# philip-bl/dctn

Hardware: AMD Instinct MI355X
Metric: EPS-contraction windows/sec (fwd+bwd) (higher is better)
Workload: dtype bf16; 1 GPU; cfg2 EPS[(3,4)]+linear bf16 B1024/GPU; parallelism=dp1

## Files before the change

### dctn_amd/_lib.py

```python
from __future__ import annotations

import ctypes
import os
import subprocess
from typing import Optional, Sequence

import torch

_HERE = os.path.dirname(os.path.abspath(__file__))
LIB_PATH = os.path.join(_HERE, "libdctn_amd.so")
CSRC = os.path.join(_HERE, "csrc")

F32, F64, BF16 = 0, 1, 2
PREC_EXACT, PREC_BF16, PREC_SPLIT, PREC_MASK = 0, 1, 2, 0xFF
OPT_F32_PREFER_HALVES, OPT_SMALL_CHUNKS, OPT_MAIN_KERNEL_ONLY, OPT_GENERIC_KERNELS = 1 << 8, 1 << 9, 1 << 10, 1 << 11
OPT_HEAD_FEATURES_BLOCKED4 = 1 << 12
ERR_BAD_SHAPE, ERR_BAD_DTYPE, ERR_UNSUPPORTED, ERR_WORKSPACE, ERR_LAUNCH, ERR_NULL = -1, -2, -3, -4, -5, -6
SAVED, PARTIAL = 1, 2
(EPS_FAMILY_GENERIC, EPS_FAMILY_Q2REG, EPS_FAMILY_BIGCORE_F32, EPS_FAMILY_HALVES, EPS_FAMILY_Q2REG_F32,
 EPS_FAMILY_BIGCORE_BF16X3) = range(6)
SBS_MATRIX_CORE_SWEEP = 1 << 8
SBS_WIDE_SWEEP = 1 << 9

_DTYPE_CODE = {torch.float32: F32, torch.float64: F64, torch.bfloat16: BF16}

c_int, c_i64, c_void, c_size = ctypes.c_int, ctypes.c_int64, ctypes.c_void_p, ctypes.c_size_t
_I64x5 = ctypes.POINTER(c_i64)
_IntP = ctypes.POINTER(c_int)
_PtrP = ctypes.POINTER(c_void)

SIGNATURES = {
    "dctn_version": (c_int, []),
    "dctn_strerror": (ctypes.c_char_p, [c_int]),
    "dctn_last_kernel": (ctypes.c_char_p, []),
    "dctn_device_limits": (c_int, [_IntP, _IntP]),
    "dctn_eps_family": (c_int, [c_int] * 9),
    "dctn_eps_fwd_workspace_bytes": (c_size, [c_int] * 7 + [c_int] * 2),
    "dctn_eps_fwd": (c_int, [c_void, _I64x5, c_void, c_void, c_void, c_size] + [c_int] * 7 + [c_int, c_int, c_void]),
    "dctn_eps_saved_bytes": (c_size, [c_int] * 7 + [c_int] * 2),
# ... 216 lines not shown
```

### dctn_amd/csrc/capi.hip

```cpp
#include "common.h"

#include <stdio.h>
#include <stdlib.h>

#include <algorithm>
#include <atomic>

static std::atomic<const char*> g_last_kernel{"none"};
void dctn_set_last_kernel(const char* name) { g_last_kernel.store(name, std::memory_order_relaxed); }

const DctnDev& dctn_dev() {
  static const DctnDev d = [] {
    DctnDev r{256, 160 * 1024};
    int dev = 0, v = 0;
    if (hipGetDevice(&dev) == hipSuccess) {
      if (hipDeviceGetAttribute(&v, hipDeviceAttributeMultiprocessorCount, dev) == hipSuccess && v > 0) r.cus = v;
      if (hipDeviceGetAttribute(&v, hipDeviceAttributeMaxSharedMemoryPerMultiprocessor, dev) == hipSuccess && v >= 64 * 1024) r.lds = v;
    }
    int cus = 0, lds = 0;
    const char* lim = getenv("DCTN_DEVICE_LIMITS");
    if (lim && sscanf(lim, "%d,%d", &cus, &lds) == 2) {
      if (cus > 0 && cus < r.cus) r.cus = cus;
      if (lds > 0 && lds < r.lds) r.lds = lds;
    }
// ... 121 lines not shown
  r.fwd_saving = r.fwd[0] == DCTN_EPS_FAMILY_Q2REG_F32 && r.saved_layout == EPS_SAVED_Z && r.saved_bytes > 0;
  r.dcore_reg = q2reg ? DCTN_EPS_FAMILY_Q2REG : q2f32 ? DCTN_EPS_FAMILY_Q2REG_F32 : EPS_NO_FAMILY;
  r.dcore_reg_saved = q2reg ? DCTN_EPS_FAMILY_Q2REG : EPS_NO_FAMILY;
  if (r.saved_layout == EPS_SAVED_HALVES)
    eps_list(r.bwd, DCTN_EPS_FAMILY_HALVES, DCTN_EPS_FAMILY_BIGCORE_F32, DCTN_EPS_FAMILY_GENERIC);
  else
    eps_list(r.bwd, DCTN_EPS_FAMILY_BIGCORE_F32, DCTN_EPS_FAMILY_GENERIC);
  return r;
}

static int eps_fwd_family(int family, const void* x, const void* core, void* out, void* ws, size_t ws_bytes, const EpsP& p,
                          int dtype, const EpsRoute& r, hipStream_t st, void* keep) {
  switch (family) {
    case DCTN_EPS_FAMILY_BIGCORE_BF16X3: return eps_fwd_bf16x3(x, core, out, ws, ws_bytes, p, dtype, DCTN_PREC_SPLIT, st, keep);
    case DCTN_EPS_FAMILY_Q2REG: return eps_fwd_mfma(x, core, out, p, dtype, r.precision, st);
    case DCTN_EPS_FAMILY_Q2REG_F32: return eps_fwd_q2f32(x, core, out, p, dtype, r.precision, st);
    case DCTN_EPS_FAMILY_BIGCORE_F32: return eps_fwd_bigcore(x, core, out, ws, ws_bytes, p, dtype, r.precision, st, keep);
    case DCTN_EPS_FAMILY_HALVES: return eps_fwd_halves(x, core, out, ws, ws_bytes, p, dtype, st, keep);
  }
  return eps_fwd_generic(x, core, out, p, dtype, st);
}

static int eps_head_params(EpsP& p, const int64_t x_strides[5], int C, int B, int H, int W, int Q, int K, int O, int Cout,
                           int dtype, int policy) {
  if (!dtype_ok(dtype)) return DCTN_ERR_BAD_DTYPE;
  if (Cout < 1) return DCTN_ERR_BAD_SHAPE;
  const int blk = policy & DCTN_OPT_HEAD_FEATURES_BLOCKED4;
  const int rc = eps_fill_params(p, x_strides, C, B, H, W, Q, K, O, policy & ~blk);
  p.opts |= blk;
  return rc;
}

static bool eps_head_next(const EpsP& p, int rc) {
  return rc == DCTN_ERR_UNSUPPORTED && !(p.opts & DCTN_OPT_HEAD_FEATURES_BLOCKED4);
}

extern "C" {

int dctn_version(void) { return 500; }

const char* dctn_last_kernel(void) { return g_last_kernel.load(std::memory_order_relaxed); }

int dctn_device_limits(int* cus, int* lds_bytes) {
  if (!cus || !lds_bytes) return DCTN_ERR_NULL;
  *cus = dctn_dev().cus;
  *lds_bytes = dctn_dev().lds;
  return DCTN_OK;
}

const char* dctn_strerror(int code) {
// ... 112 lines not shown
  if (need_dx) b = std::max(b, eps_bwd_dfactor_bigcore_workspace(p, dtype, r.precision));
  if (need_dcore) b = std::max(b, eps_bwd_dcore_bigcore_workspace(p, dtype, r.precision));
  return a + b + 256;
}

int dctn_eps_head_fwd(const void* x, const int64_t x_strides[5], const void* core, const void* head_weight,
                      const void* head_bias, void* features, void* logits, int C, int B, int H, int W, int Q, int K, int O,
                      int Cout, int dtype, int policy, void* stream) {
  if (!x || !core || !head_weight || !head_bias || !features || !logits || !x_strides) return DCTN_ERR_NULL;
  EpsP p;
  int rc = eps_head_params(p, x_strides, C, B, H, W, Q, K, O, Cout, dtype, policy);
  if (rc != DCTN_OK) return rc;
  const int precision = policy & DCTN_PREC_MASK;
  hipStream_t st = (hipStream_t)stream;
  rc = eps_head_fwd_mfma(x, core, head_weight, head_bias, features, logits, p, Cout, dtype, precision, st);
  if (!eps_head_next(p, rc)) return rc;
  return eps_head_fwd_q2f32(x, core, head_weight, head_bias, features, logits, p, Cout, dtype, precision, st);
}

size_t dctn_eps_head_bwd_workspace_bytes(int C, int B, int H, int W, int Q, int K, int O, int Cout, int dtype,
                                         int policy) {
  EpsP p;
  const int precision = policy & DCTN_PREC_MASK;
  if (!eps_query_params(p, C, B, H, W, Q, K, O, policy & ~DCTN_OPT_HEAD_FEATURES_BLOCKED4)) return 0;
  const size_t a = eps_head_bwd_mfma_workspace(p, Cout, dtype, precision), b = eps_head_bwd_q2f32_workspace(p, Cout, dtype, precision);
  return (a > b ? a : b) + 256;
}

int dctn_eps_head_bwd(const void* x, const int64_t x_strides[5], const void* features, const void* dLogits,
                      const void* head_weight, void* dCore, void* dWeight, void* dBias, void* workspace,
                      size_t workspace_bytes, int C, int B, int H, int W, int Q, int K, int O, int Cout,
                      int dtype, int policy, void* stream) {
  if (!x || !features || !dLogits || !head_weight || !dCore || !x_strides) return DCTN_ERR_NULL;
  EpsP p;
  int rc = eps_head_params(p, x_strides, C, B, H, W, Q, K, O, Cout, dtype, policy);
  if (rc != DCTN_OK) return rc;
  const int precision = policy & DCTN_PREC_MASK;
  hipStream_t st = (hipStream_t)stream;
  rc = eps_head_bwd_mfma(x, features, dLogits, head_weight, dCore, dWeight, dBias, workspace, workspace_bytes, p, Cout, dtype,
                         precision, st);
  if (!eps_head_next(p, rc)) return rc;
  return eps_head_bwd_q2f32(x, features, dLogits, head_weight, dCore, dWeight, dBias, workspace, workspace_bytes, p, Cout, dtype,
                            precision, st);
}

static int eps_bwd_impl(const void* x, const int64_t x_strides[5], const void* core, const void* dY, const void* saved,
                        size_t saved_bytes, void* dX, void* dCore, void* workspace, size_t workspace_bytes, int C, int B,
                        int H, int W, int Q, int K, int O, int dtype, int policy, void* stream) {
  if (!x || !core || !dY || !x_strides) return DCTN_ERR_NULL;
  if (!dtype_ok(dtype)) return DCTN_ERR_BAD_DTYPE;
  if (!dX && !dCore) return DCTN_OK;
  EpsP p;
  int rc = eps_fill_params(p, x_strides, C, B, H, W, Q, K, O, policy);
  if (rc != DCTN_OK) return rc;
  hipStream_t st = (hipStream_t)stream;
  const EpsRoute r = eps_route(p, dtype, policy);
  unsigned char* ws = (unsigned char*)workspace;
  size_t ws_bytes = workspace_bytes;
// ... 64 lines not shown
```

### dctn_amd/csrc/eps_generic.hip

```cpp
#include "common.h"

namespace {

template <typename S>
__device__ __forceinline__ typename AccOf<S>::type ldv(const S* p) {
  return (typename AccOf<S>::type)(*p);
}

struct WinCoord {
  long long b;
  int ho, wo;
};

__device__ __forceinline__ WinCoord win_coord(const EpsP& p, long long w) {
  WinCoord c;
  const int hw = p.Ho * p.Wo;
  c.b = w / hw;
  const int rem = (int)(w - c.b * hw);
  c.ho = rem / p.Wo;
  c.wo = rem - c.ho * p.Wo;
  return c;
}

template <typename S, typename A>
// ... 263 lines not shown
      }
    }
    if (rvalid) {
#pragma unroll
      for (int j = 0; j < OT; ++j)
        if (o0 + j < p.O) atomicAdd(&dCoreAcc[row * p.O + o0 + j], acc[j]);
    }
  }
}

}

template <typename S, typename A>
__global__ void convert_k(const A* __restrict__ src, S* __restrict__ dst, long long n) {
  for (long long i = (long long)blockIdx.x * blockDim.x + threadIdx.x; i < n;
       i += (long long)gridDim.x * blockDim.x)
    dst[i] = (S)src[i];
}
template __global__ void convert_k<bf16_t, float>(const float*, bf16_t*, long long);

int eps_fill_params(EpsP& p, const int64_t xs[5], int C, int B, int H, int W, int Q, int K, int O, int policy) {
  p.opts = policy & ~DCTN_PREC_MASK;
  if ((p.opts & ~DCTN_OPT_ALL) || (policy & DCTN_PREC_MASK) > DCTN_PREC_SPLIT || policy < 0) return DCTN_ERR_UNSUPPORTED;
  if (p.opts & DCTN_OPT_HEAD_FEATURES_BLOCKED4) return DCTN_ERR_UNSUPPORTED;
  if (C < 1 || B < 1 || Q < 1 || K < 1 || O < 1 || H < K || W < K) return DCTN_ERR_BAD_SHAPE;
  p.C = C; p.B = B; p.H = H; p.W = W; p.Q = Q; p.K = K; p.O = O;
  p.N = K * K * C;
  p.Ho = H - K + 1;
  p.Wo = W - K + 1;
  p.Wn = (long long)B * p.Ho * p.Wo;
  long long R = 1;
  for (int n = 0; n < p.N; ++n) {
    R *= Q;
    if (R > (1LL << 40)) return DCTN_ERR_UNSUPPORTED;
  }
  p.R = R;
  for (int i = 0; i < 5; ++i) p.s[i] = xs[i];
  int m = 0;
  long long lo = 1;
  while (m < p.N && lo * Q <= 32) { lo *= Q; ++m; }
  p.m = m; p.LO = (int)lo; p.NH = p.N - m;
  p.HI = ipow_ll(Q, p.NH);
  p.bits = Q <= 16 ? 4 : 8;
  return DCTN_OK;
}

static size_t fwd_lds(const EpsP& p, size_t asz) {
// ... 153 lines not shown
```

### dctn_amd/csrc/eps_mfma.hip

```cpp
#include "common.h"

#include <cstdlib>
#include <type_traits>

typedef __attribute__((ext_vector_type(8))) __bf16 bf16x8;
typedef __attribute__((ext_vector_type(16))) float f32x16;
typedef __attribute__((ext_vector_type(8))) float f32x8;
typedef __attribute__((ext_vector_type(2))) int int2v;
typedef __attribute__((ext_vector_type(4))) int int4v;
typedef __attribute__((ext_vector_type(2))) float f32x2;

namespace {

constexpr int ilog2(int v) { return v <= 1 ? 0 : 1 + ilog2(v >> 1); }

template <typename S> __device__ __forceinline__ float to_f32(S v) { return (float)v; }

__device__ __forceinline__ float half_sum(float v) {
  const int iv = __float_as_int(v);
  const int2v r = __builtin_amdgcn_permlane32_swap(iv, iv, false, false);
  return __int_as_float(r[0]) + __int_as_float(r[1]);
}

__device__ __forceinline__ void swap_halves(float& a, float& b) {
// ... 51 lines not shown
__device__ __forceinline__ unsigned fdiv(unsigned n, const FastDiv& d) {
  const unsigned t = __umulhi(d.M, n);
  return (t + ((n - t) >> d.s1)) >> d.s2;
}

#define MFMA_MAXN 16
struct MfmaP {
  int C, B, K, O, Ho, Wo;
  int P;
  int npg;
  int spc, nchunks;
  unsigned foffb[MFMA_MAXN];
  unsigned rowoffb[MFMA_MAXN];
  unsigned s1b, s2b, s3b, s4b;
  unsigned x_bytes;
  unsigned o_bytes, o_s1b;
  FastDiv div_wo;
  int rowvec_ok;
  int vec_ok;
  int Cout;
  unsigned hw_rowb, hw_bytes;
  int ncb;
  int opts;
#ifdef DCTN_STAMPS
  unsigned long long* stamps;
#endif
};

#ifdef DCTN_STAMPS
#define DCTN_STAMP(P, SLOT)                                                                      \
  do {                                                                                           \
    __builtin_amdgcn_sched_barrier(0);                                                           \
    unsigned long long t_;                                                                       \
    asm volatile("s_memrealtime %0\n\ts_waitcnt lgkmcnt(0)" : "=s"(t_)::"memory");               \
    if ((P).stamps && threadIdx.x == 0) (P).stamps[(long long)blockIdx.x * 8 + (SLOT)] = t_;     \
    __builtin_amdgcn_sched_barrier(0);                                                           \
  } while (0)
static unsigned long long* g_stamps = nullptr;
void dctn_stamps_set(unsigned long long* p) { g_stamps = p; }
__device__ unsigned long long* g_dev_stamps = nullptr;
void dctn_reduce_stamps_set(unsigned long long* p) { (void)hipMemcpyToSymbol(HIP_SYMBOL(g_dev_stamps), &p, sizeof(p)); }
#define DCTN_STAMP_T(P, SLOT, TID)                                                              \
  do {                                                                                           \
    __builtin_amdgcn_sched_barrier(0);                                                           \
    unsigned long long t_;                                                                       \
    asm volatile("s_memrealtime %0\n\ts_waitcnt lgkmcnt(0)" : "=s"(t_)::"memory");               \
// ... 178 lines not shown
        __builtin_amdgcn_raw_buffer_store_b128(u32x4{d[4 * i], d[4 * i + 1], d[4 * i + 2], d[4 * i + 3]}, rs, voff,
                                               soff + 16u * i, 0);
    }
  } else {
#pragma unroll
    for (int o = 0; o < OP; ++o)
      if (o < O) {
        if constexpr (sizeof(S) == 2)
          __builtin_amdgcn_raw_buffer_store_b16((unsigned short)(pack_bf16(v[o], 0.f) & 0xffffu), rs, voff,
                                                soff + 2u * o, 0);
        else
          __builtin_amdgcn_raw_buffer_store_b32(__float_as_uint(v[o]), rs, voff, soff + 4u * o, 0);
      }
  }
}

struct WaveJob {
  int b0, b1;
  unsigned voff_x;
  unsigned voff_o;
  int pos;
  bool valid;
};
__device__ __forceinline__ WaveJob wave_job(const MfmaP& p, int waves_per_block, int esz, bool grouped = false) {
  const int nb = gridDim.x;
  const int vb = (nb % 8 == 0) ? (int)(blockIdx.x % 8) * (nb / 8) + (int)(blockIdx.x / 8) : (int)blockIdx.x;
  const int wave = __builtin_amdgcn_readfirstlane(vb * waves_per_block + (int)(threadIdx.x >> 6));
  int chunk = wave / p.npg, pg = wave - chunk * p.npg;
  if (grouped) {
    const int cb = vb / p.npg;
    pg = vb - cb * p.npg;
    chunk = __builtin_amdgcn_readfirstlane(cb * waves_per_block + (int)(threadIdx.x >> 6));
    if (cb >= p.ncb) chunk = p.nchunks;
  }
  WaveJob j;
  j.b0 = chunk < p.nchunks ? chunk * p.spc : 0;
  j.b1 = chunk < p.nchunks ? (j.b0 + p.spc < p.B ? j.b0 + p.spc : p.B) : 0;
  j.pos = pg * 64 + (int)(threadIdx.x & 63);
  j.valid = j.pos < p.P;
  const unsigned pu = j.valid ? (unsigned)j.pos : 0u;
  const unsigned ho = fdiv(pu, p.div_wo), wo = pu - ho * (unsigned)p.Wo;
  j.voff_x = j.valid ? ho * p.s2b + wo * p.s3b : p.x_bytes;
  j.voff_o = j.valid ? pu * (unsigned)(p.O * esz) : p.o_bytes;
  return j;
}

template <int N0>
__device__ __forceinline__ void build_p0(const float (*xv)[2], bf16x8 (&X)[(1 << N0) / 16],
                                         bf16x8 (&Y)[(1 << N0) / 16]) {
// ... 540 lines not shown
      const unsigned sob = (unsigned)(g0 >> 2) * (unsigned)F * 8u;
      for (int f = 2 * tid; f < F; f += 2 * 64 * HEADT_WAVES) {
        unsigned r[HEADT_GS];
#pragma unroll
        for (int i = 0; i < HEADT_GS; ++i) r[i] = i < ng ? *reinterpret_cast<const unsigned*>(ftile + i * LP + f) : 0u;
        const u32x4 q = u32x4{__builtin_amdgcn_perm(r[1], r[0], 0x05040100u), __builtin_amdgcn_perm(r[3], r[2], 0x05040100u),
                              __builtin_amdgcn_perm(r[1], r[0], 0x07060302u), __builtin_amdgcn_perm(r[3], r[2], 0x07060302u)};
        __builtin_amdgcn_raw_buffer_store_b128(q, rs_o, (unsigned)f * 8u, sob, 0);
      }
    }
    __syncthreads();
    if (tid < HEADT_GS * 16) {
      const int sl = tid >> 4, cc = tid & 15;
      if (sl < ng && cc < p.Cout) {
        float t = (float)bias[cc];
#pragma unroll
        for (int w = 0; w < HEADT_WAVES; ++w) t += hsum[w][sl][cc];
        logits[(long long)(g0 + sl) * p.Cout + cc] = (bf16_t)t;
      }
    }
  }
}

constexpr int BWD_WAVES = 8;
constexpr size_t dcore_dyn_lds_bytes(int mt) { return (size_t)BWD_WAVES * (1 + mt) * 64 * 32 * sizeof(short); }

template <typename S, int N0, int N1, int OP, bool XVEC, bool OVEC, int ROWS, int HEADC>
__global__ __launch_bounds__(64 * BWD_WAVES) void eps_bwd_dcore_q2reg_k(const S* __restrict__ x,
                                                             const S* __restrict__ dY,
                                                             const S* __restrict__ hw,
                                                             const S* __restrict__ feat,
                                                             float* __restrict__ partial,
                                                             float* __restrict__ dwpart, MfmaP p) {
  constexpr int N = N0 + N1, A = 1 << N0, BN = 1 << N1, KS = A / 16, MT = BN * OP / 32;
  constexpr int AT = A >= 32 ? A / 32 : 1;
  constexpr int LOGO = ilog2(OP);
  constexpr bool LDST = A == 32 && MT <= 2;
  __shared__ float red[BWD_WAVES][32 * 32];
  extern __shared__ __attribute__((aligned(16))) unsigned char dsm[];
  const int tid = threadIdx.x, lane = tid & 63, r = lane & 31, h = lane >> 5, wv = tid >> 6;
  DCTN_STAMP(p, 0);
  short* tiles = reinterpret_cast<short*>(dsm) + wv * ((1 + MT) * 64 * LROW);
  const TrLane trl = tr_lane(lane);

  bf16x8 ident[2];
#pragma unroll
  for (int sp = 0; sp < 2; ++sp)
#pragma unroll
    for (int j = 0; j < 8; ++j) ident[sp][j] = (bf16_t)((16 * sp + 8 * h + j == r) ? 1.f : 0.f);

  f32x16 acc[MT][AT];
#pragma unroll
  for (int t = 0; t < MT; ++t)
#pragma unroll
    for (int a = 0; a < AT; ++a)
#pragma unroll
      for (int v = 0; v < 16; ++v) acc[t][a][v] = 0.f;

  const WaveJob job = wave_job(p, BWD_WAVES, (int)sizeof(S), HEADC > 0);
  const __amdgpu_buffer_rsrc_t rs_x = make_rsrc(x, p.x_bytes);
  const __amdgpu_buffer_rsrc_t rs_dy = make_rsrc(HEADC > 0 ? feat : dY, p.o_bytes);
  constexpr bool HEADMM = HEADC > 0 && HEADC <= 16 && LDST && OVEC && XVEC && sizeof(S) == 2 && OP == 4;
  float hwf[HEADC > 0 && !HEADMM ? HEADC : 1][OP];
  float dwacc[HEADC > 0 && !HEADMM ? HEADC : 1][OP];
#pragma unroll
  for (int c = 0; c < (HEADC > 0 && !HEADMM ? HEADC : 1); ++c)
#pragma unroll
    for (int o = 0; o < OP; ++o) dwacc[c][o] = 0.f;
  constexpr int DLW = HEADC > 0 ? HEADC / 2 : 1;
  const unsigned* dl32 = reinterpret_cast<const unsigned*>(dY);
  unsigned dlraw[DLW];
  RawRow<S, OP> rr[HEADC > 0 && !HEADMM ? HEADC : 1];
  constexpr bool LATE = HEADC > 0 && LDST && !HEADMM;
  auto issue_head_weight = [&]() {
    if constexpr (HEADC > 0 && !HEADMM) {
      const __amdgpu_buffer_rsrc_t rs_hw = make_rsrc(hw, p.hw_bytes);
      const unsigned voff_hw = job.valid ? (unsigned)job.pos * (unsigned)(OP * 2) : p.hw_bytes;
#pragma unroll
      for (int c = 0; c < HEADC; ++c)
        issue_row<S, OP, true>(rs_hw, c < p.Cout ? voff_hw : p.hw_bytes, (unsigned)c * p.hw_rowb, OP, rr[c]);
    }
  };
  auto ldst_step = [&](const float (&xv)[N][2], auto&& make_dy) {
    if constexpr (LDST) {
      bf16x8 X[KS], Y[KS];
// ... 258 lines not shown
      }
#pragma unroll
      for (int set = 0; set < 2; ++set) {
        f32x16 d;
#pragma unroll
        for (int v = 0; v < 16; ++v) d[v] = 0.f;
#pragma unroll
        for (int sp = 0; sp < 2; ++sp)
          d = __builtin_amdgcn_mfma_f32_32x32x16_bf16(zf[set][sp], ident[sp], d, 0, 0, 0);
        bf16x8 zt[2];
        zt[0] = pack8(d[0], d[1], d[2], d[3], d[4], d[5], d[6], d[7]);
        zt[1] = pack8(d[8], d[9], d[10], d[11], d[12], d[13], d[14], d[15]);
#pragma unroll
        for (int a = 0; a < AT; ++a)
#pragma unroll
          for (int s2 = 0; s2 < 2; ++s2)
            acc[t][a] = __builtin_amdgcn_mfma_f32_32x32x16_bf16(zt[s2], p0t[set][a][s2], acc[t][a], 0, 0, 0);
      }
    }
  }
  }

  DCTN_STAMP(p, 3);
  float* dst = partial + (long long)blockIdx.x * (MT * 32) * (AT * 32);
  if constexpr (LDST) {
    static_assert(AT == 1 && (size_t)BWD_WAVES * MT * 1024 * 4 <= dcore_dyn_lds_bytes(MT), "dCore tiles must fit");
    float* big = reinterpret_cast<float*>(dsm);
    DCTN_STAMP_T(p, 6, 64 * (BWD_WAVES - 1));
    __syncthreads();
    DCTN_STAMP(p, 7);
#pragma unroll
    for (int t = 0; t < MT; ++t)
#pragma unroll
      for (int v = 0; v < 16; ++v) {
        const int row = (v & 3) + 8 * (v >> 2) + 4 * h;
        big[(wv * MT + t) * 1024 + row * 32 + r] = acc[t][0][v];
      }
    __syncthreads();
    for (int e = tid; e < MT * 1024; e += 64 * BWD_WAVES) {
      float sum = 0.f;
#pragma unroll
      for (int k = 0; k < BWD_WAVES; ++k) sum += big[k * MT * 1024 + e];
      dst[e] = sum;
    }
  } else {
#pragma unroll
    for (int t = 0; t < MT; ++t)
// ... 335 lines not shown
  m.s3b = (unsigned)(p.s[3] * esz); m.s4b = (unsigned)(p.s[4] * esz);
  long long ext = 0;
  const long long dims[5] = {p.C, p.B, p.H, p.W, p.Q};
  for (int i = 0; i < 5; ++i) ext += (dims[i] - 1) * p.s[i];
  m.x_bytes = (unsigned)((ext + 1) * esz);
  const int rows = p.K * p.C;
  for (int rw = 0; rw < MFMA_MAXN; ++rw) m.rowoffb[rw] = 0;
  for (int rw = 0; rw < rows && rw < MFMA_MAXN; ++rw) {
    const int dh = rw / p.C, ch = rw - dh * p.C;
    m.rowoffb[rw] = (unsigned)((ch * p.s[0] + dh * p.s[2]) * esz);
  }
  m.rowvec_ok = dtype == DCTN_BF16 && p.s[4] == 1 && p.s[3] == 2 && p.K <= 4 && rows <= MFMA_MAXN / 2 &&
                ((p.N == 9 && rows == 3) || (p.N == 8 && rows == 4));
  m.div_wo = make_fastdiv((unsigned)p.Wo);
  m.C = p.C; m.B = p.B; m.K = p.K; m.O = p.O; m.Ho = p.Ho; m.Wo = p.Wo;
  m.P = p.Ho * p.Wo;
  m.npg = (m.P + 63) / 64;
  m.spc = 1; m.nchunks = p.B;
  m.o_s1b = (unsigned)((long long)m.P * p.O * esz);
  m.o_bytes = (unsigned)(p.Wn * p.O * esz);
  m.vec_ok = p.s[4] == 1 && p.s[0] % 2 == 0 && p.s[1] % 2 == 0 && p.s[2] % 2 == 0 &&
             p.s[3] % 2 == 0 && ((uintptr_t)x % 4) == 0;
  m.Cout = 0; m.hw_rowb = 0; m.hw_bytes = 0; m.ncb = 0;
  m.opts = p.opts;
#ifdef DCTN_STAMPS
  m.stamps = g_stamps;
#endif
}

constexpr int FWD_BLOCKS_PER_CU = 4;

template <int N0, int N1, int OP>
constexpr size_t dcore_dyn_lds() {
  constexpr int A = 1 << N0, MT = (1 << N1) * OP / 32;
  return (A == 32 && MT <= 2) ? (size_t)BWD_WAVES * (1 + MT) * 64 * LROW * sizeof(short) : 0;
}
#define DCTN_DCORE_LAUNCH(KERNEL, G, B, DYN, ST, ...)                                                  \
  do {                                                                                                 \
    if ((DYN) > 0 && !dctn_lds_optin((const void*)KERNEL, DYN)) return DCTN_ERR_UNSUPPORTED;       \
    hipLaunchKernelGGL(KERNEL, G, B, DYN, ST, __VA_ARGS__);                                            \
  } while (0)

int plan_waves(MfmaP& m, int wpb, long long target) {
  long long chunks = target / m.npg;
  if (chunks < 1) chunks = 1;
  if (chunks > m.B) chunks = m.B;
// ... 94 lines not shown
  return A == 32 && MT <= 2 && OP == 4 && m.vec_ok && blocked4_bytes(m) < (1LL << 31) && !(m.opts & DCTN_OPT_SMALL_CHUNKS) &&
         F % 8 == 0 && F <= (long long)HEADT_WAVES * HEADT_MAXKS * 32;
}

template <int N0, int N1, int OP>
int bwd_head_launch_t(const void* x, const void* dL, const void* hw, const void* feat, void* dCore, void* dW,
                      void* dBias, void* ws, size_t core_ws_bytes, const MfmaP& m_in, hipStream_t st) {
  typedef bf16_t S;
  constexpr int A = 1 << N0, BN = 1 << N1, AT = A >= 32 ? A / 32 : 1;
  constexpr size_t DYN = dcore_dyn_lds<N0, N1, OP>();
  MfmaP m = m_in;
  const bool blk = (m.opts & DCTN_OPT_HEAD_FEATURES_BLOCKED4) != 0;
  if (m.O != OP || m.Cout < 2 || m.Cout > 16 || m.Cout % 2 != 0) return DCTN_ERR_UNSUPPORTED;
  if (((uintptr_t)dL % 4) != 0 || ((uintptr_t)hw % 4) != 0 || ((uintptr_t)feat % (blk ? 16 : 4)) != 0) return DCTN_ERR_UNSUPPORTED;
  if (blk && !head_blocked4_ok<N0, N1, OP>(m)) return DCTN_ERR_UNSUPPORTED;
  const int grid = plan_grouped(m);
  if (grid == 0) return DCTN_ERR_UNSUPPORTED;
  float* dwpart = reinterpret_cast<float*>(static_cast<unsigned char*>(ws) + core_ws_bytes);
  const long long nW = (long long)m.Cout * m.P * OP;
  constexpr int MT = BN * OP / 32;
  const bool headmm = A == 32 && MT <= 2 && OP == 4 && m.vec_ok;
  if (headmm && (long long)m.B * m.P * OP * 2 >= (1LL << 31)) return DCTN_ERR_UNSUPPORTED;
  const bool gemm = headmm;

  const dim3 g(grid), b(64 * BWD_WAVES);
  constexpr int NN = N0 + N1;
  constexpr int RW = NN == 9 ? 3 : 4;
#define DCTN_HEAD_LAUNCH(XV, ROWSV, HC)                                                                        \
  DCTN_DCORE_LAUNCH((eps_bwd_dcore_q2reg_k<S, N0, N1, OP, XV, true, ROWSV, HC>), g, b, (DYN > 0 ? DYN + 8192 : 0), st, (const S*)x, \
                     (const S*)dL, (const S*)hw, (const S*)feat, (float*)ws, dwpart, m)
  if (m.rowvec_ok && m.vec_ok) {
    if (m.Cout <= 10) DCTN_HEAD_LAUNCH(true, RW, 10); else DCTN_HEAD_LAUNCH(true, RW, 16);
  } else if (m.vec_ok) {
    if (m.Cout <= 10) DCTN_HEAD_LAUNCH(true, 0, 10); else DCTN_HEAD_LAUNCH(true, 0, 16);
  } else {
    if (m.Cout <= 10) DCTN_HEAD_LAUNCH(false, 0, 10); else DCTN_HEAD_LAUNCH(false, 0, 16);
  }
#undef DCTN_HEAD_LAUNCH
  DCTN_CHECK_LAUNCH();
  if (m.opts & DCTN_OPT_MAIN_KERNEL_ONLY) return DCTN_PARTIAL;
  const int fw = blk ? DWG_BFW : DWG_FW;
  const int n_core = BN * OP * AT, n_dw = gemm ? (int)(((long long)m.P * OP + fw - 1) / fw) : (int)((nW + 255) / 256);
  const size_t gemm_lds = (size_t)DWG_WAVES * (fw / 4) * 64 * sizeof(float);
  static_assert(DWG_WAVES * 64 == 1024, "the gemm role is the whole workgroup of eps_head_reduce_k");
  if (gemm && !dctn_lds_optin((const void*)eps_head_reduce_k, gemm_lds)) return DCTN_ERR_LAUNCH;
  hipLaunchKernelGGL(eps_head_reduce_k, dim3(n_core + n_dw + 1), dim3(1024), gemm ? gemm_lds : 0, st, (const float*)ws, (S*)dCore,
                     grid, A, BN, m.O, OP, AT * 32, n_core, (const float*)dwpart, (S*)dW, m.ncb, nW, n_dw,
                     (const S*)dL, (S*)dBias, m.B, m.Cout, (const S*)feat, gemm ? (blk ? 2 : 1) : 0);
  DCTN_CHECK_LAUNCH();
  dctn_set_last_kernel("eps_head_bwd_mfma_q2reg");
  return DCTN_OK;
}

template <int N0, int N1, int OP>
int fwd_head_launch_t(const void* x, const void* core, const void* hw, const void* bias, void* out, void* logits,
                      const MfmaP& m_in, hipStream_t st) {
  typedef bf16_t S;
  MfmaP m = m_in;
  const bool blk = (m.opts & DCTN_OPT_HEAD_FEATURES_BLOCKED4) != 0;
  if (m.O != OP || !(m.rowvec_ok && m.vec_ok) || m.npg > HEAD_FWD_MAXPG) return DCTN_ERR_UNSUPPORTED;
  if (((uintptr_t)hw % 16) != 0 || m.hw_rowb % 16 != 0 || ((uintptr_t)out % (blk ? 16 : OP * 2)) != 0) return DCTN_ERR_UNSUPPORTED;
  int nwg = m.B < dctn_dev().cus ? m.B : dctn_dev().cus;
  m.spc = (m.B + nwg - 1) / nwg;
  if (blk) m.spc = (m.spc + HEADT_GS - 1) / HEADT_GS * HEADT_GS;
  nwg = (m.B + m.spc - 1) / m.spc;
  constexpr int RW = (N0 + N1) == 9 ? 3 : 4;
  const long long F = (long long)m.P * OP;
  const bool tk = !(m.opts & DCTN_OPT_SMALL_CHUNKS) && F % 8 == 0 && F <= (long long)HEADT_WAVES * HEADT_MAXKS * 32;
  if (blk) {
    if (!tk || !head_blocked4_ok<N0, N1, OP>(m)) return DCTN_ERR_UNSUPPORTED;
// ... 137 lines not shown
```

### dctn_amd/eps_plus_linear.py

```python
from __future__ import annotations

import math
from dataclasses import dataclass
from logging import getLogger
from typing import Tuple, Union

import torch
import torch.nn as nn
import torch.nn.functional as F
from torch import Tensor

from . import _lib as L
from . import eps, epses_composition
from .utils import OneTensorInitialization, ZeroCenteredNormalInitialization, ZeroCenteredUniformInitialization


@dataclass(frozen=True)
class UnitEmpiricalOutputStd:
    input: Tensor
    batch_size: int = 128


class UnitTheoreticalOutputStd:
    pass


@dataclass(frozen=True)
class ManuallyChosenInitialization:
    epses: Tuple[OneTensorInitialization, ...]
    linear_weight: OneTensorInitialization
    linear_bias: OneTensorInitialization


Initialization = Union[UnitEmpiricalOutputStd, UnitTheoreticalOutputStd, ManuallyChosenInitialization]

FUSED_HEAD = True
FUSED_HEAD_FWD = True
BLOCKED_FEATURES = True
HEAD_BWD = "hip"


class _LinearHeadFunction(torch.autograd.Function):

    @staticmethod
    def supported(feat: Tensor, weight: Tensor, bias) -> bool:
        return (
            feat.is_cuda and bias is not None and feat.dtype in (torch.bfloat16, torch.float32, torch.float64)
            and weight.dtype == feat.dtype and bias.dtype == feat.dtype and feat.ndim == 2 and weight.shape[0] <= 16
        )

    @staticmethod
    def forward(ctx, feat: Tensor, weight: Tensor, bias: Tensor) -> Tensor:
        dev = L.require_device(feat, weight, bias)
        f, w, b = feat.contiguous(), weight.contiguous(), bias.contiguous()
        B, F_ = f.shape
        C = w.shape[0]
        out = torch.empty((B, C), dtype=f.dtype, device=dev)
        L.check(L.lib().dctn_linear_head_fwd(f.data_ptr(), w.data_ptr(), b.data_ptr(), out.data_ptr(), B, F_, C,
                                             L.dtype_code(f), L.stream_ptr(dev)), "linear head forward")
        ctx.save_for_backward(f, w)
        return out
# ... 71 lines not shown
            ws = L.workspace(L.lib().dctn_eps_fwd_workspace_bytes(C, B, H, W, Q, K, O, code, prec), dev)
            L.check(
                L.lib().dctn_eps_fwd(x.data_ptr(), L.strides5(x), core_c.data_ptr(), feat.data_ptr(), ws.data_ptr(),
                                     ws.numel(), C, B, H, W, Q, K, O, code, prec, L.stream_ptr(dev)),
                "eps forward",
            )
            L.check(L.lib().dctn_linear_head_fwd(feat.data_ptr(), w.data_ptr(), b.data_ptr(), out.data_ptr(), B,
                                                 feat.shape[1], cout, code, L.stream_ptr(dev)), "linear head forward")
        else:
            L.check(rc, "eps + linear head forward")
        ctx.save_for_backward(core_c, x, feat, w)
        ctx.dims = (C, B, H, W, Q, K, O, prec)
        ctx.blocked = blocked
        return out

    @staticmethod
    def backward(ctx, d_out: Tensor):
        core_c, x, feat, w = ctx.saved_tensors
        C, B, H, W, Q, K, O, prec = ctx.dims
        need_core, _, need_w, need_b = ctx.needs_input_grad
        dev, code = x.device, L.dtype_code(x)
        g = d_out.contiguous()
        blk = L.OPT_HEAD_FEATURES_BLOCKED4 if ctx.blocked else 0

        def rows():
            return feat.permute(0, 2, 1).reshape(-1, feat.shape[1])[:B].contiguous() if ctx.blocked else feat

        if not need_core:
            _, d_w, d_b = _head_backward(rows(), w, g, False, need_w, need_b)
            return None, None, d_w, d_b
        cout = w.shape[0]
        flat = torch.empty(core_c.numel() + w.numel() + cout, dtype=w.dtype, device=dev)
        d_core = flat[: core_c.numel()].view_as(core_c)
        d_w = flat[core_c.numel() : core_c.numel() + w.numel()].view_as(w) if need_w else None
        d_b = flat[core_c.numel() + w.numel() :] if need_b else None
        nbytes = max(L.lib().dctn_eps_head_bwd_workspace_bytes(C, B, H, W, Q, K, O, cout, code, prec),
                     L.lib().dctn_eps_bwd_workspace_bytes(C, B, H, W, Q, K, O, code, prec, 0, 1))
        ws = L.workspace(nbytes, dev)
        rc = L.lib().dctn_eps_head_bwd(
            x.data_ptr(), L.strides5(x), feat.data_ptr(), g.data_ptr(), w.data_ptr(), d_core.data_ptr(),
            None if d_w is None else d_w.data_ptr(), None if d_b is None else d_b.data_ptr(), ws.data_ptr(),
            ws.numel(), C, B, H, W, Q, K, O, cout, code, prec | blk, L.stream_ptr(dev))
        if rc == L.ERR_UNSUPPORTED:
            d_feat, d_w, d_b = _head_backward(rows(), w, g, True, need_w, need_b)
            rc = L.lib().dctn_eps_bwd(x.data_ptr(), L.strides5(x), core_c.data_ptr(), d_feat.data_ptr(), None,
                                      d_core.data_ptr(), ws.data_ptr(), ws.numel(), C, B, H, W, Q, K, O, code,
# ... 132 lines not shown
```

### include/dctn_amd.h

```cpp
#ifndef DCTN_AMD_H
#define DCTN_AMD_H

#include <stddef.h>
#include <stdint.h>

#ifdef __cplusplus
extern "C" {
#endif

enum { DCTN_F32 = 0, DCTN_F64 = 1, DCTN_BF16 = 2, DCTN_DTYPE_MASK = 0xFF };
enum { DCTN_SBS_MATRIX_CORE_SWEEP = 1 << 8 };
enum { DCTN_SBS_WIDE_SWEEP = 1 << 9 };

enum {
  DCTN_OK = 0,
  DCTN_ERR_BAD_SHAPE = -1,
  DCTN_ERR_BAD_DTYPE = -2,
  DCTN_ERR_UNSUPPORTED = -3,
  DCTN_ERR_WORKSPACE = -4,
  DCTN_ERR_LAUNCH = -5,
  DCTN_ERR_NULL = -6
};
enum {
  DCTN_SAVED = 1,
  DCTN_PARTIAL = 2
};

enum {
  DCTN_PREC_EXACT = 0,
  DCTN_PREC_BF16 = 1,
  DCTN_PREC_SPLIT = 2,
  DCTN_PREC_MASK = 0xFF
};
enum {
  DCTN_OPT_F32_PREFER_HALVES = 1 << 8,
  DCTN_OPT_SMALL_CHUNKS = 1 << 9,
  DCTN_OPT_MAIN_KERNEL_ONLY = 1 << 10,
  DCTN_OPT_GENERIC_KERNELS = 1 << 11,
  DCTN_OPT_HEAD_FEATURES_BLOCKED4 = 1 << 12,
  DCTN_OPT_ALL = (1 << 8) | (1 << 9) | (1 << 10) | (1 << 11) | (1 << 12)
};

int dctn_version(void);
const char* dctn_strerror(int code);
const char* dctn_last_kernel(void);

int dctn_device_limits(int* cus, int* lds_bytes);

#define DCTN_EPS_FAMILY_GENERIC 0
#define DCTN_EPS_FAMILY_Q2REG 1
#define DCTN_EPS_FAMILY_BIGCORE_F32 2
#define DCTN_EPS_FAMILY_HALVES 3
#define DCTN_EPS_FAMILY_Q2REG_F32 4
#define DCTN_EPS_FAMILY_BIGCORE_BF16X3 5
int dctn_eps_family(int C, int B, int H, int W, int Q, int K, int O, int dtype, int policy);
size_t dctn_eps_fwd_workspace_bytes(int C, int B, int H, int W, int Q, int K, int O,
                                    int dtype, int policy);
int dctn_eps_fwd(const void* x, const int64_t x_strides[5], const void* core, void* out,
                 void* workspace, size_t workspace_bytes,
                 int C, int B, int H, int W, int Q, int K, int O,
                 int dtype, int policy, void* stream);

size_t dctn_eps_fwd_stats_workspace_bytes(int C, int B, int H, int W, int Q, int K, int O,
// ... 143 lines not shown
```

Before: 26.13 billion windows/s.

## Compute head weight gradient on idle CUs inside the dCore backward launch

When the dCore backward kernel leaves enough CUs idle, extra workgroups are appended to the grid that compute the linear head's dW via a streamed MFMA GEMM, instead of doing it in the follow-up reduce kernel. A role map assigns blocks to either dCore work or dW slices, and the reduce launch drops its dW gemm blocks. The aim is to overlap dW with the dCore pass and shorten the finish kernel. In exchange it adds LDS staging and a more complex block mapping, and a flag lets callers fall back to the old path.

```diff
diff --git a/dctn_amd/_lib.py b/dctn_amd/_lib.py
--- a/dctn_amd/_lib.py
+++ b/dctn_amd/_lib.py
@@ -15,6 +15,7 @@
 PREC_EXACT, PREC_BF16, PREC_SPLIT, PREC_MASK = 0, 1, 2, 0xFF
 OPT_F32_PREFER_HALVES, OPT_SMALL_CHUNKS, OPT_MAIN_KERNEL_ONLY, OPT_GENERIC_KERNELS = 1 << 8, 1 << 9, 1 << 10, 1 << 11
 OPT_HEAD_FEATURES_BLOCKED4 = 1 << 12
+OPT_HEAD_DW_IN_FINISH = 1 << 14
 ERR_BAD_SHAPE, ERR_BAD_DTYPE, ERR_UNSUPPORTED, ERR_WORKSPACE, ERR_LAUNCH, ERR_NULL = -1, -2, -3, -4, -5, -6
 SAVED, PARTIAL = 1, 2
 (EPS_FAMILY_GENERIC, EPS_FAMILY_Q2REG, EPS_FAMILY_BIGCORE_F32, EPS_FAMILY_HALVES, EPS_FAMILY_Q2REG_F32,
diff --git a/dctn_amd/csrc/capi.hip b/dctn_amd/csrc/capi.hip
--- a/dctn_amd/csrc/capi.hip
+++ b/dctn_amd/csrc/capi.hip
@@ -167,10 +167,10 @@
 }
 
 static int eps_head_params(EpsP& p, const int64_t x_strides[5], int C, int B, int H, int W, int Q, int K, int O, int Cout,
-                           int dtype, int policy) {
+                           int dtype, int policy, int own = 0) {
   if (!dtype_ok(dtype)) return DCTN_ERR_BAD_DTYPE;
   if (Cout < 1) return DCTN_ERR_BAD_SHAPE;
-  const int blk = policy & DCTN_OPT_HEAD_FEATURES_BLOCKED4;
+  const int blk = policy & (DCTN_OPT_HEAD_FEATURES_BLOCKED4 | own);
   const int rc = eps_fill_params(p, x_strides, C, B, H, W, Q, K, O, policy & ~blk);
   p.opts |= blk;
   return rc;
@@ -329,7 +329,7 @@
                                          int policy) {
   EpsP p;
   const int precision = policy & DCTN_PREC_MASK;
-  if (!eps_query_params(p, C, B, H, W, Q, K, O, policy & ~DCTN_OPT_HEAD_FEATURES_BLOCKED4)) return 0;
+  if (!eps_query_params(p, C, B, H, W, Q, K, O, policy & ~(DCTN_OPT_HEAD_FEATURES_BLOCKED4 | DCTN_OPT_HEAD_DW_IN_FINISH))) return 0;
   const size_t a = eps_head_bwd_mfma_workspace(p, Cout, dtype, precision), b = eps_head_bwd_q2f32_workspace(p, Cout, dtype, precision);
   return (a > b ? a : b) + 256;
 }
@@ -340,7 +340,7 @@
                       int dtype, int policy, void* stream) {
   if (!x || !features || !dLogits || !head_weight || !dCore || !x_strides) return DCTN_ERR_NULL;
   EpsP p;
-  int rc = eps_head_params(p, x_strides, C, B, H, W, Q, K, O, Cout, dtype, policy);
+  int rc = eps_head_params(p, x_strides, C, B, H, W, Q, K, O, Cout, dtype, policy, DCTN_OPT_HEAD_DW_IN_FINISH);
   if (rc != DCTN_OK) return rc;
   const int precision = policy & DCTN_PREC_MASK;
   hipStream_t st = (hipStream_t)stream;
diff --git a/dctn_amd/csrc/eps_generic.hip b/dctn_amd/csrc/eps_generic.hip
--- a/dctn_amd/csrc/eps_generic.hip
+++ b/dctn_amd/csrc/eps_generic.hip
@@ -309,7 +309,7 @@
 int eps_fill_params(EpsP& p, const int64_t xs[5], int C, int B, int H, int W, int Q, int K, int O, int policy) {
   p.opts = policy & ~DCTN_PREC_MASK;
   if ((p.opts & ~DCTN_OPT_ALL) || (policy & DCTN_PREC_MASK) > DCTN_PREC_SPLIT || policy < 0) return DCTN_ERR_UNSUPPORTED;
-  if (p.opts & DCTN_OPT_HEAD_FEATURES_BLOCKED4) return DCTN_ERR_UNSUPPORTED;
+  if (p.opts & (DCTN_OPT_HEAD_FEATURES_BLOCKED4 | DCTN_OPT_HEAD_DW_IN_FINISH)) return DCTN_ERR_UNSUPPORTED;
   if (C < 1 || B < 1 || Q < 1 || K < 1 || O < 1 || H < K || W < K) return DCTN_ERR_BAD_SHAPE;
   p.C = C; p.B = B; p.H = H; p.W = W; p.Q = Q; p.K = K; p.O = O;
   p.N = K * K * C;
diff --git a/dctn_amd/csrc/eps_mfma.hip b/dctn_amd/csrc/eps_mfma.hip
--- a/dctn_amd/csrc/eps_mfma.hip
+++ b/dctn_amd/csrc/eps_mfma.hip
@@ -97,6 +97,8 @@
   unsigned hw_rowb, hw_bytes;
   int ncb;
   int opts;
+  int dw_roles;
+  void* dw_out;
 #ifdef DCTN_STAMPS
   unsigned long long* stamps;
 #endif
@@ -321,9 +323,9 @@
   int pos;
   bool valid;
 };
-__device__ __forceinline__ WaveJob wave_job(const MfmaP& p, int waves_per_block, int esz, bool grouped = false) {
+__device__ __forceinline__ WaveJob wave_job(const MfmaP& p, int waves_per_block, int esz, bool grouped = false, int vb_in = -1) {
   const int nb = gridDim.x;
-  const int vb = (nb % 8 == 0) ? (int)(blockIdx.x % 8) * (nb / 8) + (int)(blockIdx.x / 8) : (int)blockIdx.x;
+  const int vb = vb_in >= 0 ? vb_in : (nb % 8 == 0) ? (int)(blockIdx.x % 8) * (nb / 8) + (int)(blockIdx.x / 8) : (int)blockIdx.x;
   const int wave = __builtin_amdgcn_readfirstlane(vb * waves_per_block + (int)(threadIdx.x >> 6));
   int chunk = wave / p.npg, pg = wave - chunk * p.npg;
   if (grouped) {
@@ -910,6 +912,135 @@
   }
 }
 
+constexpr int DWR_FW = 32;
+constexpr int DWR_RANGES = 16;
+constexpr int DWR_DEPTH = 12;
+constexpr int DWR_MIN_CUS = 8;
+__host__ __device__ constexpr int dwr_spw(int B) { return (((B + DWR_RANGES - 1) / DWR_RANGES) + 31) / 32 * 32; }
+__host__ __device__ constexpr size_t dwr_stage_bytes(int B) { return (size_t)16 * (DWR_RANGES * dwr_spw(B) + 8) * 2; }
+constexpr size_t DWR_JOIN_BYTES = (size_t)DWR_RANGES * 8 * 64 * sizeof(float);
+
+__device__ __forceinline__ int head_role_map(int bid, int nb, int R) {
+  const int Wk = nb - R;
+  if (Wk < 8) return bid < Wk ? bid : -1 - (bid - Wk);
+  const int x = bid & 7, i = bid >> 3;
+  const int tq = nb >> 3, tr = nb & 7, rq = R >> 3, rm = R & 7;
+  const int w_x = tq + (x < tr ? 1 : 0) - rq - (x < rm ? 1 : 0);
+  const int mt = x < tr ? x : tr, mr = x < rm ? x : rm;
+  if (i < w_x) return x * (tq - rq) + mt - mr + i;
+  return -1 - (x * rq + mr + (i - w_x));
+}
+
+__device__ __forceinline__ void head_dw_stream_role(const bf16_t* __restrict__ feat, const bf16_t* __restrict__ dL,
+                                                    bf16_t* __restrict__ dW, const MfmaP& p, int role,
+                                                    unsigned char* __restrict__ stage) {
+  typedef __attribute__((ext_vector_type(4))) float f32x4v;
+  const int tid = threadIdx.x, lane = tid & 63, wv = tid >> 6, n = lane & 15, kg = lane >> 4;
+  const int B = p.B, Cout = p.Cout;
+  const long long F = (long long)p.P * 4;
+  const int spw = dwr_spw(B), nkb = spw >> 5;
+  const int SROW = DWR_RANGES * spw + 8;
+  float* join = reinterpret_cast<float*>(stage + dwr_stage_bytes(B));
+  const int nsl = (int)((F + DWR_FW - 1) / DWR_FW);
+  const int s0 = (int)((long long)role * nsl / p.dw_roles), s1 = (int)((long long)(role + 1) * nsl / p.dw_roles);
+  const unsigned nq = (unsigned)(B + 3) >> 2;
+  const unsigned f_bytes = nq * (unsigned)F * 8u, dl_bytes = (unsigned)B * (unsigned)Cout * 2u;
+  const __amdgpu_buffer_rsrc_t rs_f = make_rsrc(feat, f_bytes), rs_dl = make_rsrc(dL, dl_bytes);
+
+  unsigned* st32 = reinterpret_cast<unsigned*>(stage);
+  const int ROWD = SROW / 2, npair = DWR_RANGES / 2 * spw;
+  auto stage_load = [&](int pi, unsigned (&r0)[8], unsigned (&r1)[8]) {
+#pragma unroll
+    for (int d = 0; d < 8; ++d) {
+      const bool c = 2 * d < Cout;
+      r0[d] = __builtin_amdgcn_raw_buffer_load_b32(rs_dl, (c && 2 * pi < B) ? (unsigned)(2 * pi) * (unsigned)Cout * 2u + 4u * d : dl_bytes, 0, 0);
+      r1[d] = __builtin_amdgcn_raw_buffer_load_b32(rs_dl, (c && 2 * pi + 1 < B) ? (unsigned)(2 * pi + 1) * (unsigned)Cout * 2u + 4u * d : dl_bytes, 0, 0);
+    }
+  };
+  auto stage_write = [&](int pi, const unsigned (&r0)[8], const unsigned (&r1)[8]) {
+#pragma unroll
+    for (int d = 0; d < 8; ++d) {
+      st32[(2 * d) * ROWD + pi] = __builtin_amdgcn_perm(r1[d], r0[d], 0x05040100u);
+      st32[(2 * d + 1) * ROWD + pi] = __builtin_amdgcn_perm(r1[d], r0[d], 0x07060302u);
+    }
+  };
+
+  int is = s0, ir = 0, ik = 0, cs = s0, cr = 0, ck = 0;
+  auto issue = [&](u32x4 (&f)[2]) {
+    const long long fcol = (long long)is * DWR_FW + 2 * n;
+    const bool fok = is < s1 && fcol + 1 < F;
+    const unsigned q0 = (unsigned)(((2 * wv + ir) * spw + 32 * ik) >> 2) + 2u * kg;
+#pragma unroll
+    for (int h = 0; h < 2; ++h) {
+      const unsigned q = q0 + h;
+      const unsigned vo = (fok && q < nq) ? (unsigned)(((long long)q * F + fcol) * 8) : f_bytes;
+      f[h] = __builtin_amdgcn_raw_buffer_load_b128(rs_f, vo, 0, 0);
+    }
+    if (++ik == nkb) {
+      ik = 0;
+      if (++ir == 2) { ir = 0; ++is; }
+    }
+  };
+  f32x4v acc[2];
+  auto consume = [&](const u32x4 (&f)[2]) {
+    const int range = 2 * wv + cr;
+    const int4v at = *reinterpret_cast<const int4v*>(stage + ((size_t)n * SROW + range * spw + 32 * ck + 8 * kg) * 2);
+    if (ck == 0) acc[0] = acc[1] = f32x4v{0.f, 0.f, 0.f, 0.f};
+#pragma unroll
+    for (int j = 0; j < 2; ++j) {
+      int4v bf;
+#pragma unroll
+      for (int d = 0; d < 4; ++d) bf[d] = (int)f[d >> 1][2 * j + (d & 1)];
+      acc[j] = __builtin_amdgcn_mfma_f32_16x16x32_bf16(__builtin_bit_cast(bf16x8, at), __builtin_bit_cast(bf16x8, bf), acc[j], 0, 0, 0);
+    }
+    if (++ck == nkb) {
+      ck = 0;
+#pragma unroll
+      for (int j = 0; j < 2; ++j)
+#pragma unroll
+        for (int i = 0; i < 4; ++i) join[(range * 8 + j * 4 + i) * 64 + lane] = acc[j][i];
+      if (++cr == 2) {
+        cr = 0;
+        __syncthreads();
+        const int slot = tid >> 6, j = slot >> 2, i = slot & 3;
+        float t = 0.f;
+#pragma unroll
+        for (int w = 0; w < DWR_RANGES; ++w) t += join[(w * 8 + slot) * 64 + lane];
+        const int c = 4 * kg + i;
+        const long long fo = (long long)cs * DWR_FW + 2 * n + j;
+        if (cs < s1 && c < Cout && fo < F) dW[(long long)c * F + fo] = (bf16_t)t;
+        ++cs;
+        __syncthreads();
+      }
+    }
+  };
+
+  unsigned r0[8], r1[8];
+  stage_load(tid, r0, r1);
+  __builtin_amdgcn_sched_barrier(0);
+  u32x4 ring[DWR_DEPTH][2];
+#pragma unroll
+  for (int u = 0; u < DWR_DEPTH; ++u) issue(ring[u]);
+  __builtin_amdgcn_sched_barrier(0);
+  if (tid < npair) stage_write(tid, r0, r1);
+  for (int pi = tid + 64 * 8; pi < npair; pi += 64 * 8) {
+    stage_load(pi, r0, r1);
+    stage_write(pi, r0, r1);
+  }
+  __syncthreads();
+  DCTN_STAMP(p, 1);
+  const int T = (s1 - s0) * 2 * nkb;
+  for (int t = 0; t < T; t += DWR_DEPTH) {
+#pragma unroll
+    for (int u = 0; u < DWR_DEPTH; ++u) {
+      consume(ring[u]);
+      issue(ring[u]);
+      if (t == 0 && u == 0) DCTN_STAMP(p, 2);
+    }
+  }
+  DCTN_STAMP(p, 6);
+}
+
 constexpr int BWD_WAVES = 8;
 constexpr size_t dcore_dyn_lds_bytes(int mt) { return (size_t)BWD_WAVES * (1 + mt) * 64 * 32 * sizeof(short); }
 
@@ -928,6 +1059,20 @@
   extern __shared__ __attribute__((aligned(16))) unsigned char dsm[];
   const int tid = threadIdx.x, lane = tid & 63, r = lane & 31, h = lane >> 5, wv = tid >> 6;
   DCTN_STAMP(p, 0);
+  constexpr bool HEADMM = HEADC > 0 && HEADC <= 16 && LDST && OVEC && XVEC && sizeof(S) == 2 && OP == 4;
+  int vb = -1;
+  if constexpr (HEADMM) {
+    static_assert(BWD_WAVES == 8 && OP == 4, "head_dw_stream_role: 8 waves of two sample ranges, 4 features per position");
+    if (p.dw_roles > 0) {
+      vb = head_role_map((int)blockIdx.x, (int)gridDim.x, p.dw_roles);
+      if (vb < 0) {
+        head_dw_stream_role(reinterpret_cast<const bf16_t*>(feat), reinterpret_cast<const bf16_t*>(dY),
+                            static_cast<bf16_t*>(p.dw_out), p, -1 - vb, dsm);
+        DCTN_STAMP(p, 5);
+        return;
+      }
+    }
+  }
   short* tiles = reinterpret_cast<short*>(dsm) + wv * ((1 + MT) * 64 * LROW);
   const TrLane trl = tr_lane(lane);
 
@@ -945,10 +1090,9 @@
 #pragma unroll
       for (int v = 0; v < 16; ++v) acc[t][a][v] = 0.f;
 
-  const WaveJob job = wave_job(p, BWD_WAVES, (int)sizeof(S), HEADC > 0);
+  const WaveJob job = wave_job(p, BWD_WAVES, (int)sizeof(S), HEADC > 0, vb);
   const __amdgpu_buffer_rsrc_t rs_x = make_rsrc(x, p.x_bytes);
   const __amdgpu_buffer_rsrc_t rs_dy = make_rsrc(HEADC > 0 ? feat : dY, p.o_bytes);
-  constexpr bool HEADMM = HEADC > 0 && HEADC <= 16 && LDST && OVEC && XVEC && sizeof(S) == 2 && OP == 4;
   float hwf[HEADC > 0 && !HEADMM ? HEADC : 1][OP];
   float dwacc[HEADC > 0 && !HEADMM ? HEADC : 1][OP];
 #pragma unroll
@@ -1253,7 +1397,11 @@
   }
 
   DCTN_STAMP(p, 3);
-  float* dst = partial + (long long)blockIdx.x * (MT * 32) * (AT * 32);
+  int tile = (int)blockIdx.x;
+  if constexpr (HEADMM) {
+    if (p.dw_roles > 0) tile = head_role_map((int)blockIdx.x, (int)gridDim.x, p.dw_roles);
+  }
+  float* dst = partial + (long long)tile * (MT * 32) * (AT * 32);
   if constexpr (LDST) {
     static_assert(AT == 1 && (size_t)BWD_WAVES * MT * 1024 * 4 <= dcore_dyn_lds_bytes(MT), "dCore tiles must fit");
     float* big = reinterpret_cast<float*>(dsm);
@@ -1635,6 +1783,7 @@
   m.vec_ok = p.s[4] == 1 && p.s[0] % 2 == 0 && p.s[1] % 2 == 0 && p.s[2] % 2 == 0 &&
              p.s[3] % 2 == 0 && ((uintptr_t)x % 4) == 0;
   m.Cout = 0; m.hw_rowb = 0; m.hw_bytes = 0; m.ncb = 0;
+  m.dw_roles = 0; m.dw_out = nullptr;
   m.opts = p.opts;
 #ifdef DCTN_STAMPS
   m.stamps = g_stamps;
@@ -1775,8 +1924,16 @@
   const bool headmm = A == 32 && MT <= 2 && OP == 4 && m.vec_ok;
   if (headmm && (long long)m.B * m.P * OP * 2 >= (1LL << 31)) return DCTN_ERR_UNSUPPORTED;
   const bool gemm = headmm;
-
-  const dim3 g(grid), b(64 * BWD_WAVES);
+  const int working = m.ncb * m.npg;
+  if (headmm && blk && dW && !(m.opts & DCTN_OPT_HEAD_DW_IN_FINISH) && dctn_dev().cus - working >= DWR_MIN_CUS &&
+      dwr_stage_bytes(m.B) + DWR_JOIN_BYTES <= DYN + 8192) {
+    const int slices = (int)(((long long)m.P * OP + DWR_FW - 1) / DWR_FW), free_cus = dctn_dev().cus - working;
+    m.dw_roles = free_cus < slices ? free_cus : slices;
+    m.dw_out = dW;
+  }
+  const int nblk = m.dw_roles > 0 ? working : grid;
+
+  const dim3 g(m.dw_roles > 0 ? working + m.dw_roles : grid), b(64 * BWD_WAVES);
   constexpr int NN = N0 + N1;
   constexpr int RW = NN == 9 ? 3 : 4;
 #define DCTN_HEAD_LAUNCH(XV, ROWSV, HC)                                                                        \
@@ -1793,12 +1950,14 @@
   DCTN_CHECK_LAUNCH();
   if (m.opts & DCTN_OPT_MAIN_KERNEL_ONLY) return DCTN_PARTIAL;
   const int fw = blk ? DWG_BFW : DWG_FW;
-  const int n_core = BN * OP * AT, n_dw = gemm ? (int)(((long long)m.P * OP + fw - 1) / fw) : (int)((nW + 255) / 256);
+  const int n_core = BN * OP * AT;
+  const int n_dw = m.dw_roles > 0 ? 0 : gemm ? (int)(((long long)m.P * OP + fw - 1) / fw) : (int)((nW + 255) / 256);
   const size_t gemm_lds = (size_t)DWG_WAVES * (fw / 4) * 64 * sizeof(float);
   static_assert(DWG_WAVES * 64 == 1024, "the gemm role is the whole workgroup of eps_head_reduce_k");
+  static_assert(DWR_RANGES == DWG_WAVES, "the in-launch role splits the samples as the gemm role does (same bits)");
   if (gemm && !dctn_lds_optin((const void*)eps_head_reduce_k, gemm_lds)) return DCTN_ERR_LAUNCH;
-  hipLaunchKernelGGL(eps_head_reduce_k, dim3(n_core + n_dw + 1), dim3(1024), gemm ? gemm_lds : 0, st, (const float*)ws, (S*)dCore,
-                     grid, A, BN, m.O, OP, AT * 32, n_core, (const float*)dwpart, (S*)dW, m.ncb, nW, n_dw,
+  hipLaunchKernelGGL(eps_head_reduce_k, dim3(n_core + n_dw + 1), dim3(1024), gemm && n_dw ? gemm_lds : 0, st, (const float*)ws, (S*)dCore,
+                     nblk, A, BN, m.O, OP, AT * 32, n_core, (const float*)dwpart, (S*)dW, m.ncb, nW, n_dw,
                      (const S*)dL, (S*)dBias, m.B, m.Cout, (const S*)feat, gemm ? (blk ? 2 : 1) : 0);
   DCTN_CHECK_LAUNCH();
   dctn_set_last_kernel("eps_head_bwd_mfma_q2reg");
diff --git a/dctn_amd/eps_plus_linear.py b/dctn_amd/eps_plus_linear.py
--- a/dctn_amd/eps_plus_linear.py
+++ b/dctn_amd/eps_plus_linear.py
@@ -37,6 +37,7 @@
 FUSED_HEAD = True
 FUSED_HEAD_FWD = True
 BLOCKED_FEATURES = True
+HEAD_DW_IN_LAUNCH = True
 HEAD_BWD = "hip"
 
 
@@ -154,6 +155,8 @@
         dev, code = x.device, L.dtype_code(x)
         g = d_out.contiguous()
         blk = L.OPT_HEAD_FEATURES_BLOCKED4 if ctx.blocked else 0
+        if not HEAD_DW_IN_LAUNCH:
+            blk |= L.OPT_HEAD_DW_IN_FINISH
 
         def rows():
             return feat.permute(0, 2, 1).reshape(-1, feat.shape[1])[:B].contiguous() if ctx.blocked else feat
diff --git a/include/dctn_amd.h b/include/dctn_amd.h
--- a/include/dctn_amd.h
+++ b/include/dctn_amd.h
@@ -38,7 +38,8 @@
   DCTN_OPT_MAIN_KERNEL_ONLY = 1 << 10,
   DCTN_OPT_GENERIC_KERNELS = 1 << 11,
   DCTN_OPT_HEAD_FEATURES_BLOCKED4 = 1 << 12,
-  DCTN_OPT_ALL = (1 << 8) | (1 << 9) | (1 << 10) | (1 << 11) | (1 << 12)
+  DCTN_OPT_HEAD_DW_IN_FINISH = 1 << 14,
+  DCTN_OPT_ALL = (1 << 8) | (1 << 9) | (1 << 10) | (1 << 11) | (1 << 12) | (1 << 14)
 };
 
 int dctn_version(void);
```

Result: slower. 23.06 billion windows/s (-11.7%).
